# heliaxdev/ark-plonk

Measured on AMD Instinct MI355X. Metric: proofs/sec at 2^20 constraints (BLS12-381, KZG10); MSM G1-adds/s, higher is better.
Workload: dtype u32 limbs (256/384-bit Montgomery integers)

## Files before the change

### ark_plonk_amd/csrc/fieldu.cuh

```cuda
#pragma once
#include "zk_common.h"

template <class P>
struct Fu {
    static constexpr int NL = P::NL;
    static constexpr int SAT = P::SAT_WORDS;
    static constexpr uint32_t M = (1u << 29) - 1u;
    uint32_t v[NL];

    ZK_HD static Fu zero() {
        Fu r;
#pragma unroll
        for (int i = 0; i < NL; ++i) r.v[i] = 0;
        return r;
    }
    ZK_HD static Fu one() {
        Fu r;
#pragma unroll
        for (int i = 0; i < NL; ++i) r.v[i] = P::ONE(i);
        return r;
    }
    ZK_HD bool limbs_zero() const {
        uint32_t o = 0;
#pragma unroll
        for (int i = 0; i < NL; ++i) o |= v[i];
        return o == 0;
    }

    ZK_HD static void normalize(Fu& t) {
#pragma unroll
        for (int i = 0; i < NL - 1; ++i) {
            uint32_t c = (uint32_t)((int32_t)t.v[i] >> 29);
            t.v[i] &= M;
            t.v[i + 1] += c;
        }
    }

    ZK_HD static Fu add(const Fu& a, const Fu& b) {
        Fu t;
#pragma unroll
        for (int i = 0; i < NL; ++i) t.v[i] = a.v[i] + b.v[i];
        normalize(t);
        return t;
    }
    ZK_HD static Fu dbl(const Fu& a) {
        Fu t;
#pragma unroll
        for (int i = 0; i < NL; ++i) t.v[i] = a.v[i] << 1;
        normalize(t);
        return t;
    }
    ZK_HD static Fu add3(const Fu& a, const Fu& b, const Fu& c) {
        Fu t;
#pragma unroll
        for (int i = 0; i < NL; ++i) t.v[i] = a.v[i] + b.v[i] + c.v[i];
        normalize(t);
        return t;
    }
    ZK_HD static Fu sub2(const Fu& a, const Fu& b) {
        Fu t;
#pragma unroll
        for (int i = 0; i < NL; ++i) t.v[i] = a.v[i] - b.v[i] + P::Z2(i);
        normalize(t);
        return t;
    }
    ZK_HD static Fu sub8(const Fu& a, const Fu& b) {
        Fu t;
#pragma unroll
        for (int i = 0; i < NL; ++i) t.v[i] = a.v[i] - b.v[i] + P::Z8(i);
        normalize(t);
        return t;
    }
    ZK_HD static Fu sub16(const Fu& a, const Fu& b) {
        Fu t;
#pragma unroll
        for (int i = 0; i < NL; ++i) t.v[i] = a.v[i] - b.v[i] + P::Z16(i);
        normalize(t);
        return t;
    }
    ZK_HD static Fu neg16(const Fu& a) {
        Fu t;
#pragma unroll
        for (int i = 0; i < NL; ++i) t.v[i] = P::Z16(i) - a.v[i];
        normalize(t);
        return t;
    }
    ZK_HD static Fu neg_canonical(const Fu& a) {
        Fu t;
#pragma unroll
        for (int i = 0; i < NL; ++i) t.v[i] = P::ZP(i) - a.v[i];
        normalize(t);
        return t;
    }

    ZK_HD static void sweep(Fu& t) {
#pragma unroll
        for (int i = 0; i < NL - 1; ++i) {
            const uint32_t c = t.v[i] >> 29;
            t.v[i] &= M;
            t.v[i + 1] += c;
        }
    }
    ZK_HD static Fu add_raw(const Fu& a, const Fu& b) {
        Fu t;
#pragma unroll
        for (int i = 0; i < NL; ++i) t.v[i] = a.v[i] + b.v[i];
        return t;
    }
    ZK_HD static Fu sub_raw3(const Fu& a, const Fu& b) {
        Fu t;
#pragma unroll
        for (int i = 0; i < NL; ++i) t.v[i] = a.v[i] + P::ZB3(i) - b.v[i];
        return t;
    }
    ZK_HD static Fu sub_raw8(const Fu& a, const Fu& b) {
        Fu t;
#pragma unroll
        for (int i = 0; i < NL; ++i) t.v[i] = a.v[i] + P::ZB8(i) - b.v[i];
        return t;
    }
    ZK_HD static Fu sub_raw16(const Fu& a, const Fu& b) {
        Fu t;
#pragma unroll
        for (int i = 0; i < NL; ++i) t.v[i] = a.v[i] + P::ZB16(i) - b.v[i];
        return t;
    }

    ZK_HD static Fu mul(const Fu& a, const Fu& b) {
        uint32_t m[NL];
        Fu r;
        uint64_t carry = 0;
#pragma unroll
        for (int k = 0; k < NL; ++k) {
            uint64_t a0 = 0, a1 = 0, am = 0;
#pragma unroll
            for (int i = 0; i <= k; ++i) {
                if (i & 1) a1 += (uint64_t)a.v[i] * b.v[k - i];
                else a0 += (uint64_t)a.v[i] * b.v[k - i];
            }
#pragma unroll
            for (int i = 0; i < k; ++i) am += (uint64_t)m[i] * P::MOD(k - i);
            uint64_t t = a0 + a1 + am + carry;
            m[k] = ((uint32_t)t * P::PINV) & M;
            t += (uint64_t)m[k] * P::MOD(0);
            carry = t >> 29;
        }
#pragma unroll
        for (int k = NL; k < 2 * NL - 1; ++k) {
            uint64_t a0 = 0, a1 = 0, am = 0;
#pragma unroll
            for (int i = k - NL + 1; i < NL; ++i) {
                if (i & 1) a1 += (uint64_t)a.v[i] * b.v[k - i];
                else a0 += (uint64_t)a.v[i] * b.v[k - i];
                am += (uint64_t)m[i] * P::MOD(k - i);
            }
            uint64_t t = a0 + a1 + am + carry;
            r.v[k - NL] = (uint32_t)t & M;
            carry = t >> 29;
        }
        r.v[NL - 1] = (uint32_t)carry;
        return r;
    }
    ZK_HD static uint64_t fence64(uint64_t t) {
#if defined(__HIP_DEVICE_COMPILE__)
        asm("" : "+v"(t));
#endif
        return t;
    }
    ZK_HD static Fu mul_fenced(const Fu& a, const Fu& b) {
        uint32_t m[NL];
        Fu r;
        uint64_t carry = 0;
#pragma unroll
        for (int k = 0; k < NL; ++k) {
            uint64_t t = fence64(carry + (uint64_t)a.v[0] * b.v[k]);
#pragma unroll
            for (int i = 1; i <= k; ++i) t += (uint64_t)a.v[i] * b.v[k - i];
#pragma unroll
            for (int i = 0; i < k; ++i) t += (uint64_t)m[i] * P::MOD(k - i);
            m[k] = ((uint32_t)t * P::PINV) & M;
            t += (uint64_t)m[k] * P::MOD(0);
            carry = t >> 29;
        }
#pragma unroll
        for (int k = NL; k < 2 * NL - 1; ++k) {
            uint64_t t = fence64(carry + (uint64_t)a.v[k - NL + 1] * b.v[NL - 1]);
#pragma unroll
            for (int i = k - NL + 2; i < NL; ++i) t += (uint64_t)a.v[i] * b.v[k - i];
#pragma unroll
            for (int i = k - NL + 1; i < NL; ++i) t += (uint64_t)m[i] * P::MOD(k - i);
            r.v[k - NL] = (uint32_t)t & M;
            carry = t >> 29;
        }
        r.v[NL - 1] = (uint32_t)carry;
        return r;
    }
    ZK_HD static Fu sqr(const Fu& a) {
        uint32_t m[NL], a2[NL];
        Fu r;
#pragma unroll
        for (int i = 0; i < NL; ++i) a2[i] = a.v[i] << 1;
        uint64_t carry = 0;
#pragma unroll
        for (int k = 0; k < NL; ++k) {
            uint64_t aa = 0, am = 0;
#pragma unroll
            for (int i = 0; 2 * i < k; ++i) aa += (uint64_t)a2[i] * a.v[k - i];
            if ((k & 1) == 0) aa += (uint64_t)a.v[k / 2] * a.v[k / 2];
#pragma unroll
            for (int i = 0; i < k; ++i) am += (uint64_t)m[i] * P::MOD(k - i);
            uint64_t t = aa + am + carry;
            m[k] = ((uint32_t)t * P::PINV) & M;
            t += (uint64_t)m[k] * P::MOD(0);
            carry = t >> 29;
        }
#pragma unroll
        for (int k = NL; k < 2 * NL - 1; ++k) {
            uint64_t aa = 0, am = 0;
#pragma unroll
            for (int i = k - NL + 1; 2 * i < k; ++i) aa += (uint64_t)a2[i] * a.v[k - i];
            if ((k & 1) == 0) aa += (uint64_t)a.v[k / 2] * a.v[k / 2];
#pragma unroll
            for (int i = k - NL + 1; i < NL; ++i) am += (uint64_t)m[i] * P::MOD(k - i);
            uint64_t t = aa + am + carry;
            r.v[k - NL] = (uint32_t)t & M;
            carry = t >> 29;
        }
        r.v[NL - 1] = (uint32_t)carry;
        return r;
    }

    ZK_HD bool is_zero_mod_reduced() const {
        if (v[0] != 0 && v[0] != P::MOD(0)) return false;
        uint32_t dz = 0, dp = 0;
#pragma unroll
        for (int i = 0; i < NL; ++i) {
            dz |= v[i];
            dp |= v[i] ^ P::MOD(i);
        }
        return dz == 0 || dp == 0;
    }
    ZK_HD bool is_zero_mod() const { return mul(*this, one()).is_zero_mod_reduced(); }

    ZK_HD static Fu canonical_lt2p(const Fu& a) {
        Fu d;
#pragma unroll
        for (int i = 0; i < NL; ++i) d.v[i] = a.v[i] - P::MOD(i);
        normalize(d);
        const bool neg = ((int32_t)d.v[NL - 1]) < 0;
        Fu r;
#pragma unroll
        for (int i = 0; i < NL; ++i) r.v[i] = neg ? a.v[i] : d.v[i];
        return r;
    }

    ZK_HD static Fu from_sat(const uint32_t* w) {
        Fu t = split_words(w);
        Fu c;
#pragma unroll
        for (int i = 0; i < NL; ++i) c.v[i] = P::C_IN(i);
        return mul(t, c);
    }
    ZK_HD void to_sat(uint32_t* w) const {
        Fu c;
#pragma unroll
        for (int i = 0; i < NL; ++i) c.v[i] = P::C_OUT(i);
        Fu t = canonical_lt2p(mul(*this, c));
        t.pack_words(w);
    }
    ZK_HD static Fu split_words(const uint32_t* w) {
        Fu t;
#pragma unroll
        for (int i = 0; i < NL; ++i) {
            const int bit = 29 * i;
            const int wi = bit >> 5, off = bit & 31;
            uint64_t lo = wi < SAT ? w[wi] : 0u;
            uint64_t hi = (wi + 1) < SAT ? w[wi + 1] : 0u;
            t.v[i] = (uint32_t)(((hi << 32) | lo) >> off) & M;
        }
        return t;
    }
    ZK_HD void pack_words(uint32_t* w) const {
#pragma unroll
        for (int j = 0; j < SAT; ++j) {
            const int lo_bit = 32 * j;
            uint64_t acc = 0;
#pragma unroll
            for (int i = 0; i < NL; ++i) {
                const int lb = 29 * i;
                if (lb + 29 <= lo_bit || lb >= lo_bit + 32) continue;
                if (lb >= lo_bit) acc |= (uint64_t)v[i] << (lb - lo_bit);
                else acc |= (uint64_t)v[i] >> (lo_bit - lb);
            }
            w[j] = (uint32_t)acc;
        }
    }

    ZK_HD static Fu pow_words(const Fu& a, const uint32_t* e, int n) {
        Fu r = one();
        bool started = false;
        for (int i = n - 1; i >= 0; --i)
            for (int b = 31; b >= 0; --b) {
                if (started) r = sqr(r);
                if ((e[i] >> b) & 1u) {
                    r = mul(r, a);
                    started = true;
                }
            }
        return r;
    }
    ZK_HD static Fu inverse(const Fu& a) {
        Fu pm;
#pragma unroll
        for (int i = 0; i < NL; ++i) pm.v[i] = P::MOD(i);
        uint32_t e[SAT];
        pm.pack_words(e);
        uint64_t t = (uint64_t)e[0] - 2u;
        e[0] = (uint32_t)t;
        uint32_t borrow = (uint32_t)(t >> 32) & 1u;
        for (int i = 1; i < SAT && borrow; ++i) {
            t = (uint64_t)e[i] - borrow;
            e[i] = (uint32_t)t;
            borrow = (uint32_t)(t >> 32) & 1u;
        }
        return pow_words(a, e, SAT);
    }
};
```

### ark_plonk_amd/csrc/ntt.hip

```cpp
#include "ctx.h"

#include "ntt_pass.cuh"

namespace {

template <class Fr>
ZK_D Fr ld_fr(const void* base, uint64_t idx) {
    const uint4* q = reinterpret_cast<const uint4*>(base) + 2 * idx;
    uint4 a = q[0], b = q[1];
    Fr r;
    r.v[0] = a.x; r.v[1] = a.y; r.v[2] = a.z; r.v[3] = a.w;
    r.v[4] = b.x; r.v[5] = b.y; r.v[6] = b.z; r.v[7] = b.w;
    return r;
}
template <class Fr>
ZK_D void st_fr(void* base, uint64_t idx, const Fr& r) {
    uint4* q = reinterpret_cast<uint4*>(base) + 2 * idx;
    q[0] = make_uint4(r.v[0], r.v[1], r.v[2], r.v[3]);
    q[1] = make_uint4(r.v[4], r.v[5], r.v[6], r.v[7]);
}

template <class Fr>
struct PowBits {
    Fr p[32];
};
template <class Fr>
__global__ void gen_pow_table(void* out, uint64_t n, PowBits<Fr> pb, Fr mul, int mode, uint32_t log_m, uint32_t log_mprev, Fr to_rp) {
    uint64_t i = (uint64_t)blockIdx.x * blockDim.x + threadIdx.x;
    if (i >= n) return;
    uint64_t e = i;
    if (mode == 1) {
        uint64_t col = i & ((1ull << log_m) - 1);
        uint64_t k = i >> log_m;
        e = (col * k) & ((1ull << log_mprev) - 1);
    }
    Fr r = mul;
    for (int b = 0; b < 32; ++b) {
        if ((e >> b) & 1ull) r = Fr::mul(r, pb.p[b]);
    }
    st_fr<Fr>(out, i, Fr::mul(r, to_rp));
}

template <class FU>
__global__ void split_table(const void* packed, void* out, uint64_t n) {
    const uint64_t i = (uint64_t)blockIdx.x * blockDim.x + threadIdx.x;
    if (i >= n) return;
    const FU x = ld_u<FU>(packed, i);
    uint32_t w[4 * TW_INNER_U4];
#pragma unroll
    for (int k = 0; k < 4 * TW_INNER_U4; ++k) w[k] = k < FU::NL ? x.v[k] : 0u;
    uint4* q = reinterpret_cast<uint4*>(out) + TW_INNER_U4 * i;
#pragma unroll
    for (int k = 0; k < TW_INNER_U4; ++k) q[k] = make_uint4(w[4 * k], w[4 * k + 1], w[4 * k + 2], w[4 * k + 3]);
}

template <class Fr>
__global__ void ntt_tiny(const void* in, void* out, uint64_t in_len, uint32_t log_n, Fr w , Fr pre_g ,
                         Fr post_g , Fr scale ) {
    if (threadIdx.x != 0 || blockIdx.x != 0) return;
    const uint32_t n = 1u << log_n;
    Fr x[4], y[4];
    Fr gp = Fr::one();
    for (uint32_t i = 0; i < n; ++i) {
        x[i] = i < in_len ? Fr::mul(ld_fr<Fr>(in, i), gp) : Fr::zero();
        gp = Fr::mul(gp, pre_g);
    }
    Fr wi = Fr::one(), pg = scale;
    for (uint32_t i = 0; i < n; ++i) {
        Fr acc = Fr::zero(), wij = Fr::one();
        for (uint32_t j = 0; j < n; ++j) {
            acc = Fr::add(acc, Fr::mul(x[j], wij));
            wij = Fr::mul(wij, wi);
        }
        y[i] = Fr::mul(acc, pg);
        pg = Fr::mul(pg, post_g);
        wi = Fr::mul(wi, w);
    }
    for (uint32_t i = 0; i < n; ++i) st_fr<Fr>(out, i, y[i]);
}

template <class Fr>
__global__ void fr_convert_kernel(const void* in, void* out, uint64_t n, int to_mont) {
    uint64_t i = (uint64_t)blockIdx.x * blockDim.x + threadIdx.x;
    if (i >= n) return;
    Fr x = ld_fr<Fr>(in, i);
    st_fr<Fr>(out, i, to_mont ? Fr::to_mont(x) : Fr::from_mont(x));
}
template <class Fr>
__global__ void fr_mul_kernel(const void* a, const void* b, void* out, uint64_t n) {
    uint64_t i = (uint64_t)blockIdx.x * blockDim.x + threadIdx.x;
    if (i >= n) return;
    st_fr<Fr>(out, i, Fr::mul(ld_fr<Fr>(a, i), ld_fr<Fr>(b, i)));
}

template <class C>
typename C::Fr root_of_unity_host(uint32_t log_n) {
    typedef typename C::Fr Fr;
    Fr r;
    for (int i = 0; i < Fr::N; ++i) r.v[i] = C::FrP::ROOT(i);
    for (uint32_t k = log_n; k < (uint32_t)C::FrP::TWO_ADICITY; ++k) r = Fr::sqr(r);
    return r;
}

template <class Fr>
PowBits<Fr> make_powbits(Fr base) {
    PowBits<Fr> pb;
    Fr cur = base;
    for (int b = 0; b < 32; ++b) {
        pb.p[b] = cur;
        cur = Fr::sqr(cur);
    }
    return pb;
}

template <class C>
typename C::Fr rprime_plain() {
    typename C::Fr r;
    C::FrU::one().pack_words(r.v);
    return r;
}

template <class C>
int launch_pow_table(zk_ctx* c, void* out, uint64_t n, typename C::Fr base, typename C::Fr mul, int mode, uint32_t log_m,
                     uint32_t log_mprev) {
    typedef typename C::Fr Fr;
    if (n == 0) return ZK_OK;
    PowBits<Fr> pb = make_powbits(base);
    Fr to_rp = rprime_plain<C>();
    const int T = 256;
    uint64_t blocks = (n + T - 1) / T;
    hipLaunchKernelGGL(gen_pow_table<Fr>, dim3((unsigned)blocks), dim3(T), 0, c->stream, out, n, pb, mul, mode, log_m, log_mprev, to_rp);
    ZK_HIP_TRY(hipGetLastError());
    return ZK_OK;
}

void decompose(uint32_t log_n, int& n_pass, int s[4]) {
    s[0] = s[1] = s[2] = s[3] = 0;
    if (log_n <= 9) {
        n_pass = 1;
        s[0] = (int)log_n;
        return;
    }
    n_pass = (int)((log_n + 8) / 9);
    int base = (int)log_n / n_pass, extra = (int)log_n % n_pass;
    for (int i = 0; i < n_pass; ++i) s[i] = base + (i < extra ? 1 : 0);
}

template <class C>
int get_inner_tw(zk_ctx* c, int s, bool inverse, void** out) {
    typedef typename C::Fr Fr;
    uint64_t key = ((uint64_t)C::ID << 40) | ((uint64_t)(inverse ? 1 : 0) << 32) | (uint64_t)s;
    auto it = c->inner_tw.find(key);
    if (it != c->inner_tw.end()) {
        *out = it->second;
        return ZK_OK;
    }
    uint64_t cnt = s >= 1 ? (1ull << (s - 1)) : 1;
    void* packed = nullptr;
    void* p = nullptr;
    ZK_HIP_TRY(hipMalloc(&packed, cnt * sizeof(Fr)));
    if (hipMalloc(&p, cnt * TW_INNER_U4 * 16) != hipSuccess) {
        (void)hipFree(packed);
        return ZK_ERR_OOM;
    }
    Fr w = root_of_unity_host<C>((uint32_t)s);
    if (inverse) w = Fr::inverse(w);
    int rc = launch_pow_table<C>(c, packed, cnt, w, Fr::one(), 0, 0, 0);
    if (!rc) {
        const int T = 256;
        hipLaunchKernelGGL(split_table<typename C::FrU>, dim3((unsigned)((cnt + T - 1) / T)), dim3(T), 0, c->stream, packed, p, cnt);
        if (hipGetLastError() != hipSuccess || hipStreamSynchronize(c->stream) != hipSuccess) rc = ZK_ERR_HIP;
    }
    (void)hipFree(packed);
    if (rc) {
        (void)hipFree(p);
        return rc;
    }
    c->inner_tw[key] = p;
    *out = p;
    return ZK_OK;
}

template <class C>
int get_plan(zk_ctx* c, uint32_t log_n, bool inverse, NttPlan** out) {
    typedef typename C::Fr Fr;
    uint64_t key = ((uint64_t)C::ID << 40) | ((uint64_t)(inverse ? 1 : 0) << 32) | log_n;
    auto it = c->plans.find(key);
    if (it != c->plans.end()) {
        *out = it->second;
        return ZK_OK;
    }
    NttPlan* pl = new NttPlan();
    pl->curve = C::ID;
    pl->log_n = log_n;
    pl->inverse = inverse;
    decompose(log_n, pl->n_pass, pl->s);
    uint32_t log_mprev = log_n;
    for (int p = 0; p < pl->n_pass; ++p) {
        if (log_n >= 3) {
            int rc = get_inner_tw<C>(c, pl->s[p], inverse, &pl->tw_inner[p]);
            if (rc) { delete pl; return rc; }
        }
        if (p + 1 < pl->n_pass) {
            uint32_t log_m = log_mprev - (uint32_t)pl->s[p];
            uint64_t cnt = 1ull << log_mprev;
            hipError_t e = hipMalloc(&pl->tw_pass[p], cnt * sizeof(Fr));
            if (e != hipSuccess) { delete pl; return ZK_ERR_OOM; }
            Fr w = root_of_unity_host<C>(log_mprev);
            if (inverse) w = Fr::inverse(w);
            int rc = launch_pow_table<C>(c, pl->tw_pass[p], cnt, w, Fr::one(), 1, log_m, log_mprev);
            if (rc) { delete pl; return rc; }
            log_mprev = log_m;
        }
    }
    c->plans[key] = pl;
    *out = pl;
    return ZK_OK;
}

template <class C>
int ensure_coset(zk_ctx* c, bool inv, uint64_t len, void** out) {
    typedef typename C::Fr Fr;
    DevBuf& buf = inv ? c->coset_inv_pow[C::ID] : c->coset_pow[C::ID];
    size_t& have = inv ? c->coset_inv_len[C::ID] : c->coset_len[C::ID];
    if (have < len) {
        ZK_HIP_TRY(hipStreamSynchronize(c->stream));
        uint64_t want = 1;
        while (want < len) want <<= 1;
        int rc = buf.ensure(want * sizeof(Fr));
        if (rc) return rc;
        Fr g = Fr::from_u32(C::FrP::GENERATOR);
        if (inv) g = Fr::inverse(g);
        rc = launch_pow_table<C>(c, buf.p, want, g, Fr::one(), 0, 0, 0);
        if (rc) return rc;
        have = want;
    }
    *out = buf.p;
    return ZK_OK;
}

typedef int (*NttPassLauncher)(int final_pass, const NttPassArgs* a, hipStream_t st);
extern "C" NttPassLauncher zk_ntt_pass_launcher(int curve, int s);

template <class C>
int dispatch_pass(zk_ctx* c, int s, bool final_pass, const NttPassArgs& a) {
    if (s < 3 || s > 9) return ZK_ERR_UNSUPPORTED;
    NttPassLauncher fn = zk_ntt_pass_launcher(C::ID, s);
    if (!fn) return ZK_ERR_UNSUPPORTED;
    hipError_t e = (hipError_t)fn(final_pass ? 1 : 0, &a, c->stream);
    ZK_HIP_TRY(e);
    return ZK_OK;
}

template <class C>
int ntt_run(zk_ctx* c, int kind, uint32_t log_n, uint32_t n_polys, const void* const* d_ins, const size_t* in_lens, void* const* d_outs) {
    typedef typename C::Fr Fr;
    if (log_n > (uint32_t)C::FrP::TWO_ADICITY) return ZK_ERR_DOMAIN_TOO_LARGE;
    if (n_polys == 0 || n_polys > 16) return ZK_ERR_BAD_ARG;
    const uint64_t N = 1ull << log_n;
    size_t in_len = 0;
    bool all_quarter = true;
    for (uint32_t i = 0; i < n_polys; ++i) {
        if (in_lens[i] > N) return ZK_ERR_BAD_ARG;
        if (in_lens[i] > in_len) in_len = in_lens[i];
        if ((uint64_t)in_lens[i] * 4 > N) all_quarter = false;
    }
    const void* d_in = d_ins[0];
    void* d_out = d_outs[0];
    const bool inverse = (kind == ZK_NTT_IFFT || kind == ZK_NTT_COSET_IFFT);
    int rc;
    Fr n_inv = Fr::inverse(Fr::from_u64(N));
    if (log_n < 3) {
        Fr w = root_of_unity_host<C>(log_n);
        if (inverse) w = Fr::inverse(w);
        Fr g = Fr::from_u32(C::FrP::GENERATOR);
        Fr pre_g = kind == ZK_NTT_COSET_FFT ? g : Fr::one();
        Fr post_g = kind == ZK_NTT_COSET_IFFT ? Fr::inverse(g) : Fr::one();
        ProfScope ps(c, "ntt_pass");
        for (uint32_t i = 0; i < n_polys; ++i)
            hipLaunchKernelGGL(ntt_tiny<Fr>, dim3(1), dim3(64), 0, c->stream, d_ins[i], d_outs[i], (uint64_t)in_lens[i], log_n, w, pre_g, post_g,
                               inverse ? n_inv : Fr::one());
        ZK_HIP_TRY(hipGetLastError());
        return ZK_OK;
    }
    void* pre = nullptr;
    void* post = nullptr;
    if (kind == ZK_NTT_COSET_FFT && in_len > 0) {
        rc = ensure_coset<C>(c, false, in_len, &pre);
        if (rc) return rc;
    }
    if (kind == ZK_NTT_COSET_IFFT) {
        rc = ensure_coset<C>(c, true, N, &post);
        if (rc) return rc;
    }
    NttPlan* pl = nullptr;
    rc = get_plan<C>(c, log_n, inverse, &pl);
    if (rc) return rc;
    if (pl->n_pass > 4) return ZK_ERR_UNSUPPORTED;
    void* work = nullptr;
    if (pl->n_pass > 1) {
        rc = c->ntt_work.ensure((size_t)n_polys * N * sizeof(Fr));
        if (rc) return rc;
        work = c->ntt_work.p;
    }
    const Fr to_rp = rprime_plain<C>();
    uint32_t log_mprev = log_n;
    NttPassArgs a;
    ProfScope ps(c, "ntt_pass");
    for (int p = 0; p < pl->n_pass; ++p) {
        const int s = pl->s[p];
        const bool last = (p + 1 == pl->n_pass);
        memset(&a, 0, sizeof a);
        a.log_n = log_n;
        a.in = (p == 0) ? d_in : work;
        a.out = last ? d_out : work;
        a.in_len = (p == 0) ? in_lens[0] : N;
        if (n_polys > 1) {
            a.n_batch = n_polys;
            for (uint32_t i = 0; i < n_polys; ++i) {
                void* wk = (char*)work + (size_t)i * N * sizeof(Fr);
                a.ins[i] = (p == 0) ? d_ins[i] : wk;
                a.outs[i] = last ? d_outs[i] : wk;
                a.in_lens[i] = (p == 0) ? in_lens[i] : N;
            }
        }
        a.tw_inner = pl->tw_inner[p];
        a.pre_mul = (p == 0) ? pre : nullptr;
        const uint32_t LC = 9u - (uint32_t)s;
        if (!last) {
            uint32_t log_m = log_mprev - (uint32_t)s;
            uint32_t logc = LC < log_m ? LC : log_m;
            a.logc = logc;
            a.log_m = log_m;
            a.log_mprev = log_mprev;
            a.tw_pass = pl->tw_pass[p];
            a.n_tiles = (uint32_t)(N >> ((uint32_t)s + logc));
            a.quarter = (p == 0 && s >= 3 && all_quarter) ? 1u : 0u;
            log_mprev = log_m;
        } else {
            uint32_t s1 = (pl->n_pass > 1) ? (uint32_t)pl->s[0] : 0;
            uint32_t logc = LC < s1 ? LC : s1;
            a.logc = logc;
            a.s1 = s1;
            a.s2 = pl->n_pass == 4 ? (uint32_t)pl->s[1] : 0u;
            a.post_mul = post;
            Fr sc = Fr::mul(inverse ? n_inv : Fr::one(), to_rp);
            for (int i = 0; i < 8; ++i) a.scale[i] = sc.v[i];
            a.n_tiles = (uint32_t)(N >> ((uint32_t)s + logc));
        }
        rc = dispatch_pass<C>(c, s, last, a);
        if (rc) return rc;
    }
    return ZK_OK;
}

}

int ntt_run_dev(zk_ctx* c, int curve, int kind, uint32_t log_n, const void* d_in, size_t in_len, void* d_out) {
    return ntt_run_batch_dev(c, curve, kind, log_n, 1, &d_in, &in_len, &d_out);
}

int ntt_run_batch_dev(zk_ctx* c, int curve, int kind, uint32_t log_n, uint32_t n_polys, const void* const* d_ins, const size_t* in_lens,
                      void* const* d_outs) {
    if (kind < 0 || kind > 3) return ZK_ERR_BAD_ARG;
    for (uint32_t base = 0; base < n_polys; base += 16) {
        const uint32_t cnt = n_polys - base < 16 ? n_polys - base : 16;
        const int rc = zk_on_curve(curve, ZK_ERR_BAD_ARG, [&](auto cv) {
            return ntt_run<decltype(cv)>(c, kind, log_n, cnt, d_ins + base, in_lens + base, d_outs + base);
        });
        if (rc) return rc;
    }
    return ZK_OK;
}

int ntt_prepare(zk_ctx* c, int curve, uint32_t log_n) {
    NttPlan* pl;
    if (log_n < 3) return ZK_OK;
    for (int inv = 0; inv < 2; ++inv) {
        const int rc = zk_on_curve(curve, ZK_ERR_BAD_ARG, [&](auto cv) {
            typedef decltype(cv) Cv;
            if (log_n > (uint32_t)Cv::FrP::TWO_ADICITY) return ZK_ERR_DOMAIN_TOO_LARGE;
            return get_plan<Cv>(c, log_n, inv != 0, &pl);
        });
        if (rc) return rc;
    }
    return ZK_OK;
}

void ntt_ctx_free(zk_ctx* c) {
    for (auto& kv : c->plans) delete kv.second;
    c->plans.clear();
    for (auto& kv : c->inner_tw) (void)hipFree(kv.second);
    c->inner_tw.clear();
    c->ntt_work.release();
    for (int i = 0; i < 2; ++i) {
        c->coset_pow[i].release();
        c->coset_inv_pow[i].release();
    }
}

static int fr_convert_on(int curve, int to_mont, const void* d_in, size_t n, void* d_out, hipStream_t st) {
    if (n == 0) return ZK_OK;
    const int T = 256;
    unsigned blocks = (unsigned)((n + T - 1) / T);
    const int rc = zk_on_curve(curve, ZK_ERR_BAD_ARG, [&](auto cv) {
        hipLaunchKernelGGL(fr_convert_kernel<typename decltype(cv)::Fr>, dim3(blocks), dim3(T), 0, st, d_in, d_out, (uint64_t)n, to_mont);
        return ZK_OK;
    });
    if (rc) return rc;
    ZK_HIP_TRY(hipGetLastError());
    return ZK_OK;
}
int fr_convert_dev(zk_ctx* c, int curve, int to_mont, const void* d_in, size_t n, void* d_out) {
    return fr_convert_on(curve, to_mont, d_in, n, d_out, c->stream);
}
int fr_convert_stream(zk_ctx* c, int curve, const void* d_in, size_t n, void* d_out, hipStream_t st) {
    (void)c;
    return fr_convert_on(curve, 0, d_in, n, d_out, st);
}

int fr_mul_dev(zk_ctx* c, int curve, const void* a, const void* b, size_t n, void* out) {
    if (n == 0) return ZK_OK;
    const int T = 256;
    unsigned blocks = (unsigned)((n + T - 1) / T);
    const int rc = zk_on_curve(curve, ZK_ERR_BAD_ARG, [&](auto cv) {
        hipLaunchKernelGGL(fr_mul_kernel<typename decltype(cv)::Fr>, dim3(blocks), dim3(T), 0, c->stream, a, b, out, (uint64_t)n);
        return ZK_OK;
    });
    if (rc) return rc;
    ZK_HIP_TRY(hipGetLastError());
    return ZK_OK;
}
```

### ark_plonk_amd/csrc/ntt_pass.cuh

```cuda
#pragma once
#include <hip/hip_runtime.h>
#include "curve_params.h"
#include "field.cuh"
#include "fieldu.cuh"

typedef __attribute__((address_space(3))) volatile uint32_t lds_u32;

struct NttPassArgs {
    const void* in;
    void* out;
    const void* tw_inner;
    const void* tw_pass;
    const void* pre_mul;
    const void* post_mul;
    uint32_t scale[8];
    uint64_t in_len;
    uint32_t log_n;
    uint32_t logc;
    uint32_t log_m;
    uint32_t log_mprev;
    uint32_t s1;
    uint32_t s2;
    uint32_t n_tiles;
    uint32_t quarter;
    uint32_t n_batch;
    const void* ins[16];
    void* outs[16];
    uint64_t in_lens[16];
};

__host__ __device__ inline uint32_t bitrev32(uint32_t x, int bits) {
#if defined(__HIP_DEVICE_COMPILE__)
    return bits ? __brev(x) >> (32 - bits) : 0u;
#else
    uint32_t r = 0;
    for (int i = 0; i < bits; ++i) { r = (r << 1) | (x & 1); x >>= 1; }
    return r;
#endif
}

template <class F>
ZK_D F ld_u(const void* base, uint64_t idx) {
    const uint4* q = reinterpret_cast<const uint4*>(base) + 2 * idx;
    uint4 a = q[0], b = q[1];
    uint32_t w[8] = {a.x, a.y, a.z, a.w, b.x, b.y, b.z, b.w};
    return F::split_words(w);
}
template <class F>
ZK_D void st_u(void* base, uint64_t idx, const F& x) {
    uint32_t w[8];
    F::canonical_lt2p(x).pack_words(w);
    uint4* q = reinterpret_cast<uint4*>(base) + 2 * idx;
    q[0] = make_uint4(w[0], w[1], w[2], w[3]);
    q[1] = make_uint4(w[4], w[5], w[6], w[7]);
}

template <class F>
ZK_D void st_u_raw(void* base, uint64_t idx, const F& x) {
    uint32_t w[8];
    x.pack_words(w);
    uint4* q = reinterpret_cast<uint4*>(base) + 2 * idx;
    q[0] = make_uint4(w[0], w[1], w[2], w[3]);
    q[1] = make_uint4(w[4], w[5], w[6], w[7]);
}

constexpr int TW_INNER_U4 = 3;
template <class F>
ZK_D F ld_limbs(const void* base, uint64_t idx) {
    static_assert(F::NL <= 4 * TW_INNER_U4, "inner twiddle entry too small");
    const uint4* q = reinterpret_cast<const uint4*>(base) + TW_INNER_U4 * idx;
    F r;
#pragma unroll
    for (int i = 0; i < TW_INNER_U4; ++i) {
        if (4 * i >= F::NL) break;
        const uint4 a = q[i];
        if (4 * i + 0 < F::NL) r.v[4 * i + 0] = a.x;
        if (4 * i + 1 < F::NL) r.v[4 * i + 1] = a.y;
        if (4 * i + 2 < F::NL) r.v[4 * i + 2] = a.z;
        if (4 * i + 3 < F::NL) r.v[4 * i + 3] = a.w;
    }
    return r;
}

constexpr int ntt_units_before(int t) {
    int b = 1;
    for (int s = 0; s < t; ++s) {
        if (b > 6) b = 1;
        b += 2;
    }
    return b;
}
constexpr bool ntt_sweep_at(int t) { return ntt_units_before(t) > 6; }
static_assert(ntt_units_before(1) == 3 && ntt_units_before(2) == 5 && ntt_units_before(3) == 7 && ntt_units_before(4) == 3, "two units per stage");
static_assert(!ntt_sweep_at(0) && !ntt_sweep_at(2) && ntt_sweep_at(3) && !ntt_sweep_at(5) && ntt_sweep_at(6) && ntt_sweep_at(9), "a sweep every third stage");

template <int B0>
ZK_D uint32_t window_pos(uint32_t v, uint32_t e) {
    return ((v >> B0) << (B0 + 3)) | (e << B0) | (v & ((1u << B0) - 1u));
}

template <class F>
ZK_D void wave_exchange(F (&x)[8], lds_u32* sc, const uint32_t (&widx)[8], const uint32_t (&ridx)[8]) {
#pragma unroll
    for (int l = 0; l < F::NL; ++l) {
#pragma unroll
        for (int e = 0; e < 8; ++e) sc[widx[e]] = x[e].v[l];
        __builtin_amdgcn_wave_barrier();
#pragma unroll
        for (int e = 0; e < 8; ++e) x[e].v[l] = sc[ridx[e]];
        __builtin_amdgcn_wave_barrier();
    }
}

template <class F, int S, int B0, int LB_LO, int LB_HI>
ZK_D void dit_window(F (&x)[8], uint32_t v, const void* tw, bool quarter) {
    const uint32_t vlow = v & ((1u << B0) - 1u);
#pragma unroll
    for (int lb = LB_LO; lb < LB_HI; ++lb) {
        const int t = B0 + lb;
        if (ntt_sweep_at(t)) {
#pragma unroll
            for (int e = 0; e < 8; ++e) F::sweep(x[e]);
        }
#pragma unroll
        for (int e = 0; e < 8; ++e) {
            if (e & (1 << lb)) continue;
            const int eo = e | (1 << lb);
            if constexpr (B0 == 0 && LB_LO == 0) {
                if (lb < 2 && quarter) {
                    x[eo] = x[e];
                    continue;
                }
                if (lb == 0) {
                    const F b = x[eo];
                    x[eo] = F::sub_raw3(x[e], b);
                    x[e] = F::add_raw(x[e], b);
                    continue;
                }
                if ((e & ((1 << lb) - 1)) == 0) {
                    F b = x[eo];
                    F::sweep(b);
                    x[eo] = lb == 1 ? F::sub_raw8(x[e], b) : F::sub_raw16(x[e], b);
                    x[e] = F::add_raw(x[e], b);
                    continue;
                }
            }
            const uint32_t plow = ((uint32_t)(e & ((1 << lb) - 1)) << B0) | vlow;
            const uint32_t j = plow << (S - 1 - t);
            F w = ld_limbs<F>(tw, j);
            F m = F::mul_fenced(x[eo], w);
            x[eo] = F::sub_raw3(x[e], m);
            x[e] = F::add_raw(x[e], m);
        }
    }
}

template <class F, int S, int B0>
ZK_D void dit_all(F (&x)[8], uint32_t v, uint32_t c, uint32_t LC, const void* tw, lds_u32* sc, bool quarter = false) {
    constexpr int REM = S - B0;
    if constexpr (REM >= 3) {
        dit_window<F, S, B0, 0, 3>(x, v, tw, quarter);
        if constexpr (REM > 3) {
            constexpr int NB0 = (REM - 3 >= 3) ? B0 + 3 : S - 3;
            uint32_t wi[8], ri[8];
#pragma unroll
            for (int e = 0; e < 8; ++e) {
                wi[e] = (window_pos<B0>(v, e) << LC) | c;
                ri[e] = (window_pos<NB0>(v, e) << LC) | c;
            }
            wave_exchange<F>(x, sc, wi, ri);
            if constexpr (REM - 3 >= 3) {
                dit_all<F, S, B0 + 3>(x, v, c, LC, tw, sc);
            } else {
                dit_window<F, S, S - 3, 3 - (REM - 3), 3>(x, v, tw, false);
            }
        }
    }
}

template <class F, int S>
__global__ void __launch_bounds__(256) ntt_pass_mid(NttPassArgs a) {
    constexpr uint32_t LC = 9 - S;
    __shared__ uint32_t scratch[4][512];
    const uint32_t lane = threadIdx.x & 63, wv = threadIdx.x >> 6;
    const uint32_t tile = blockIdx.x * (blockDim.x >> 6) + wv;
    if (tile >= a.n_tiles) return;
    const void* in = a.in;
    void* out = a.out;
    uint64_t in_len = a.in_len;
    if (a.n_batch) {
        in = a.ins[blockIdx.y];
        out = a.outs[blockIdx.y];
        in_len = a.in_lens[blockIdx.y];
    }
    lds_u32* sc = (lds_u32*)scratch[wv];
    const uint32_t c = lane & ((1u << LC) - 1u);
    const uint32_t v = lane >> LC;
    const bool active = c < (1u << a.logc);
    const uint32_t lcg = a.log_m - a.logc;
    const uint64_t blk = (uint64_t)tile >> lcg;
    const uint64_t cg = (uint64_t)tile & ((1ull << lcg) - 1);
    const uint64_t col = (cg << a.logc) + c;
    const uint64_t base = (blk << a.log_mprev) + col;

    F x[8];
#pragma unroll
    for (int e = 0; e < 8; ++e) {
        const uint64_t row = bitrev32((v << 3) | e, S);
        const uint64_t idx = base + (row << a.log_m);
        if (active && idx < in_len) {
            x[e] = ld_u<F>(in, idx);
            if (a.pre_mul) x[e] = F::mul_fenced(x[e], ld_u<F>(a.pre_mul, idx));
        } else {
            x[e] = F::zero();
        }
    }
    dit_all<F, S, 0>(x, v, c, LC, a.tw_inner, sc, a.quarter != 0);
    if (!active) return;
#pragma unroll
    for (int e = 0; e < 8; ++e) {
        const uint64_t k = S >= 3 ? (((uint64_t)e << (S - 3)) | v) : e;
        F w = ld_u<F>(a.tw_pass, (k << a.log_m) + col);
        if (ntt_units_before(S) > 6) F::sweep(x[e]);
        st_u_raw<F>(out, base + (k << a.log_m), F::mul_fenced(x[e], w));
    }
}

template <class F, int S>
__global__ void __launch_bounds__(256) ntt_pass_final(NttPassArgs a) {
    constexpr uint32_t L = 1u << S;
    constexpr uint32_t LC = 9 - S;
    __shared__ uint32_t scratch[4][512];
    const uint32_t lane = threadIdx.x & 63, wv = threadIdx.x >> 6;
    const uint32_t tile = blockIdx.x * (blockDim.x >> 6) + wv;
    if (tile >= a.n_tiles) return;
    const void* in = a.in;
    void* out = a.out;
    uint64_t in_len = a.in_len;
    if (a.n_batch) {
        in = a.ins[blockIdx.y];
        out = a.outs[blockIdx.y];
        in_len = a.in_lens[blockIdx.y];
    }
    lds_u32* sc = (lds_u32*)scratch[wv];
    const uint32_t log_nb = a.log_n - S;
    const uint32_t log_rest = log_nb - a.s1;
    const uint32_t lg = a.s1 - a.logc;
    const uint64_t rho = (uint64_t)tile >> lg;
    const uint64_t g = (uint64_t)tile & ((1ull << lg) - 1);

    F x[8];
    uint32_t wi[8], ri[8];
    const uint32_t c = lane & ((1u << LC) - 1u);
    const uint32_t v = lane >> LC;
#pragma unroll
    for (int e = 0; e < 8; ++e) {
        const uint32_t q = (uint32_t)e * 64u + lane;
        const uint32_t cb = q >> S, row = q & (L - 1);
        const uint64_t b = ((((uint64_t)g << a.logc) + cb) << log_rest) | rho;
        const uint64_t idx = (b << S) + row;
        if (cb < (1u << a.logc) && idx < in_len) {
            x[e] = ld_u<F>(in, idx);
            if (a.pre_mul) x[e] = F::mul_fenced(x[e], ld_u<F>(a.pre_mul, idx));
        } else {
            x[e] = F::zero();
        }
        wi[e] = (bitrev32(row, S) << LC) | cb;
        ri[e] = (((v << 3) | (uint32_t)e) << LC) | c;
    }
    wave_exchange<F>(x, sc, wi, ri);
    dit_all<F, S, 0>(x, v, c, LC, a.tw_inner, sc);
    if (c >= (1u << a.logc)) return;
    const uint64_t k1o = ((uint64_t)g << a.logc) + c;
    uint64_t rho_rev = rho;
    if (a.s2) {
        const uint32_t s3 = log_rest - a.s2;
        rho_rev = (rho >> s3) | ((rho & ((1ull << s3) - 1ull)) << a.s2);
    }
    const uint64_t obase = k1o + (rho_rev << a.s1);
    F sc_mul = F::split_words(a.scale);
#pragma unroll
    for (int e = 0; e < 8; ++e) {
        const uint64_t k = S >= 3 ? (((uint64_t)e << (S - 3)) | v) : e;
        const uint64_t oidx = obase + (k << log_nb);
        if (ntt_units_before(S) > 6) F::sweep(x[e]);
        F y = F::mul_fenced(x[e], sc_mul);
        if (a.post_mul) y = F::mul_fenced(y, ld_u<F>(a.post_mul, oidx));
        st_u<F>(out, oidx, y);
    }
}
```

### ark_plonk_amd/csrc/ntt_pass_inst.hip

```cpp
#include "ntt_pass.cuh"

#if ZK_CURVE_SEL == 0
typedef Fu<FrBls12_381UParams> FrSel;
#define ZK_LAUNCHER_NAME2(s) zk_ntt_pass_c0_s##s
#else
typedef Fu<FrBn254UParams> FrSel;
#define ZK_LAUNCHER_NAME2(s) zk_ntt_pass_c1_s##s
#endif
#define ZK_LAUNCHER_NAME(s) ZK_LAUNCHER_NAME2(s)

extern "C" int ZK_LAUNCHER_NAME(ZK_NTT_S)(int final_pass, const NttPassArgs* a, hipStream_t st) {
    constexpr int S = ZK_NTT_S;
    const unsigned waves = a->n_tiles < 4 ? a->n_tiles : 4;
    const unsigned blocks = (a->n_tiles + waves - 1) / waves;
    const unsigned polys = a->n_batch ? a->n_batch : 1;
    if (final_pass)
        hipLaunchKernelGGL((ntt_pass_final<FrSel, S>), dim3(blocks, polys), dim3(64 * waves), 0, st, *a);
    else
        hipLaunchKernelGGL((ntt_pass_mid<FrSel, S>), dim3(blocks, polys), dim3(64 * waves), 0, st, *a);
    return (int)hipGetLastError();
}
```

Before: 12.79.

## Fold inverse-NTT scale into mid-pass twiddles and skip final-pass scale multiply

```diff
diff --git a/ark_plonk_amd/csrc/fieldu.cuh b/ark_plonk_amd/csrc/fieldu.cuh
--- a/ark_plonk_amd/csrc/fieldu.cuh
+++ b/ark_plonk_amd/csrc/fieldu.cuh
@@ -253,6 +253,24 @@
         for (int i = 0; i < NL; ++i) r.v[i] = neg ? a.v[i] : d.v[i];
         return r;
     }
+
+    ZK_HD static Fu reduce_lt47p(const Fu& a) {
+        constexpr uint32_t T = P::MOD(NL - 1) + 1u;
+        static_assert(P::MOD(NL - 1) >= (1u << 20) && 47ull * T < (1ull << 29), "quotient estimate: top limb of p out of range");
+        constexpr uint32_t QM = (uint32_t)((1ull << 35) / T);
+        const uint32_t q = (uint32_t)(((uint64_t)a.v[NL - 1] * QM) >> 35);
+        Fu d;
+        int64_t c = 0;
+#pragma unroll
+        for (int i = 0; i < NL - 1; ++i) {
+            const int64_t t = c + (int64_t)a.v[i] - (int64_t)((uint64_t)q * P::MOD(i));
+            d.v[i] = (uint32_t)t & M;
+            c = t >> 29;
+        }
+        d.v[NL - 1] = (uint32_t)c + a.v[NL - 1] - q * P::MOD(NL - 1);
+        return d;
+    }
+    ZK_HD static Fu canonical_lt47p(const Fu& a) { return canonical_lt2p(reduce_lt47p(a)); }
 
     ZK_HD static Fu from_sat(const uint32_t* w) {
         Fu t = split_words(w);
diff --git a/ark_plonk_amd/csrc/ntt.hip b/ark_plonk_amd/csrc/ntt.hip
--- a/ark_plonk_amd/csrc/ntt.hip
+++ b/ark_plonk_amd/csrc/ntt.hip
@@ -208,7 +208,9 @@
             if (e != hipSuccess) { delete pl; return ZK_ERR_OOM; }
             Fr w = root_of_unity_host<C>(log_mprev);
             if (inverse) w = Fr::inverse(w);
-            int rc = launch_pow_table<C>(c, pl->tw_pass[p], cnt, w, Fr::one(), 1, log_m, log_mprev);
+            const bool fold = inverse && p + 2 == pl->n_pass;
+            int rc = launch_pow_table<C>(c, pl->tw_pass[p], cnt, w, fold ? Fr::inverse(Fr::from_u64(1ull << log_n)) : Fr::one(), 1, log_m,
+                                         log_mprev);
             if (rc) { delete pl; return rc; }
             log_mprev = log_m;
         }
@@ -239,15 +241,15 @@
     return ZK_OK;
 }
 
-typedef int (*NttPassLauncher)(int final_pass, const NttPassArgs* a, hipStream_t st);
+typedef int (*NttPassLauncher)(int pass, const NttPassArgs* a, hipStream_t st);
 extern "C" NttPassLauncher zk_ntt_pass_launcher(int curve, int s);
 
 template <class C>
-int dispatch_pass(zk_ctx* c, int s, bool final_pass, const NttPassArgs& a) {
+int dispatch_pass(zk_ctx* c, int s, int pass, const NttPassArgs& a) {
     if (s < 3 || s > 9) return ZK_ERR_UNSUPPORTED;
     NttPassLauncher fn = zk_ntt_pass_launcher(C::ID, s);
     if (!fn) return ZK_ERR_UNSUPPORTED;
-    hipError_t e = (hipError_t)fn(final_pass ? 1 : 0, &a, c->stream);
+    hipError_t e = (hipError_t)fn(pass, &a, c->stream);
     ZK_HIP_TRY(e);
     return ZK_OK;
 }
@@ -344,11 +346,13 @@
             a.s1 = s1;
             a.s2 = pl->n_pass == 4 ? (uint32_t)pl->s[1] : 0u;
             a.post_mul = post;
-            Fr sc = Fr::mul(inverse ? n_inv : Fr::one(), to_rp);
-            for (int i = 0; i < 8; ++i) a.scale[i] = sc.v[i];
+            if (pl->n_pass == 1) {
+                Fr sc = Fr::mul(inverse ? n_inv : Fr::one(), to_rp);
+                for (int i = 0; i < 8; ++i) a.scale[i] = sc.v[i];
+            }
             a.n_tiles = (uint32_t)(N >> ((uint32_t)s + logc));
         }
-        rc = dispatch_pass<C>(c, s, last, a);
+        rc = dispatch_pass<C>(c, s, !last ? 0 : pl->n_pass == 1 ? 1 : 2, a);
         if (rc) return rc;
     }
     return ZK_OK;
diff --git a/ark_plonk_amd/csrc/ntt_pass.cuh b/ark_plonk_amd/csrc/ntt_pass.cuh
--- a/ark_plonk_amd/csrc/ntt_pass.cuh
+++ b/ark_plonk_amd/csrc/ntt_pass.cuh
@@ -226,7 +226,7 @@
     }
 }
 
-template <class F, int S>
+template <class F, int S, bool SCALE>
 __global__ void __launch_bounds__(256) ntt_pass_final(NttPassArgs a) {
     constexpr uint32_t L = 1u << S;
     constexpr uint32_t LC = 9 - S;
@@ -278,14 +278,26 @@
         rho_rev = (rho >> s3) | ((rho & ((1ull << s3) - 1ull)) << a.s2);
     }
     const uint64_t obase = k1o + (rho_rev << a.s1);
-    F sc_mul = F::split_words(a.scale);
+    F sc_mul;
+    if constexpr (SCALE) sc_mul = F::split_words(a.scale);
 #pragma unroll
     for (int e = 0; e < 8; ++e) {
         const uint64_t k = S >= 3 ? (((uint64_t)e << (S - 3)) | v) : e;
         const uint64_t oidx = obase + (k << log_nb);
-        if (ntt_units_before(S) > 6) F::sweep(x[e]);
-        F y = F::mul_fenced(x[e], sc_mul);
-        if (a.post_mul) y = F::mul_fenced(y, ld_u<F>(a.post_mul, oidx));
-        st_u<F>(out, oidx, y);
-    }
-}
+        if constexpr (SCALE) {
+            if (ntt_units_before(S) > 6) F::sweep(x[e]);
+            F y = F::mul_fenced(x[e], sc_mul);
+            if (a.post_mul) y = F::mul_fenced(y, ld_u<F>(a.post_mul, oidx));
+            st_u<F>(out, oidx, y);
+        } else {
+            F y;
+            if (a.post_mul) {
+                if (ntt_units_before(S) > 6) F::sweep(x[e]);
+                y = F::mul_fenced(x[e], ld_u<F>(a.post_mul, oidx));
+            } else {
+                y = F::reduce_lt47p(x[e]);
+            }
+            st_u<F>(out, oidx, y);
+        }
+    }
+}
diff --git a/ark_plonk_amd/csrc/ntt_pass_inst.hip b/ark_plonk_amd/csrc/ntt_pass_inst.hip
--- a/ark_plonk_amd/csrc/ntt_pass_inst.hip
+++ b/ark_plonk_amd/csrc/ntt_pass_inst.hip
@@ -9,13 +9,18 @@
 #endif
 #define ZK_LAUNCHER_NAME(s) ZK_LAUNCHER_NAME2(s)
 
-extern "C" int ZK_LAUNCHER_NAME(ZK_NTT_S)(int final_pass, const NttPassArgs* a, hipStream_t st) {
+extern "C" int ZK_LAUNCHER_NAME(ZK_NTT_S)(int pass, const NttPassArgs* a, hipStream_t st) {
     constexpr int S = ZK_NTT_S;
     const unsigned waves = a->n_tiles < 4 ? a->n_tiles : 4;
     const unsigned blocks = (a->n_tiles + waves - 1) / waves;
     const unsigned polys = a->n_batch ? a->n_batch : 1;
-    if (final_pass)
-        hipLaunchKernelGGL((ntt_pass_final<FrSel, S>), dim3(blocks, polys), dim3(64 * waves), 0, st, *a);
+    if (pass == 2) {
+        if constexpr (S >= 5)
+            hipLaunchKernelGGL((ntt_pass_final<FrSel, S, false>), dim3(blocks, polys), dim3(64 * waves), 0, st, *a);
+        else
+            return (int)hipErrorInvalidValue;
+    } else if (pass == 1)
+        hipLaunchKernelGGL((ntt_pass_final<FrSel, S, true>), dim3(blocks, polys), dim3(64 * waves), 0, st, *a);
     else
         hipLaunchKernelGGL((ntt_pass_mid<FrSel, S>), dim3(blocks, polys), dim3(64 * waves), 0, st, *a);
     return (int)hipGetLastError();
```

New measurement: 12.76. No clear change (-0.2%).
